# hhergeth/CudaTracerLib

Measured on AMD Instinct MI355X. Metric: Mrays/s at 1920x1080, 267 spp (steps), depth-8; achieved HBM GB/s vs peak, higher is better.
Workload: dtype f32; 1 GPU; synthetic-SM 1920x1080, 1 spp/step, depth 8, NEE on, 2000 instances x icosphere(4)/boxes, 8631000 instanced triangles; rough_transmittance=the reference's 3-D lookup on every call (bit-equal frames), framebuffer_reduce=none (1 GPU)

## Files before the change

cudatracerlib_amd/build.py:

```python
import hashlib, os, subprocess, sys, glob, tempfile

HERE = os.path.dirname(os.path.abspath(__file__))
CSRC = os.path.join(HERE, "csrc")
OUT = os.path.join(HERE, "libctl_amd.so")
SRCS = ["kernels.hip", "shade_basic.hip", "shade_full.hip", "shade_class_a.hip", "shade_class_b.hip", "shade_class_c.hip", "shade_class_p.hip", "shade_class_g.hip", "shade_class_g_wf.hip", "shade_class_p_wf.hip", "shade_class_a_wf.hip", "shade_class_b_wf.hip", "shade_class_c_wf.hip", "shade_basic_wf.hip", "shade_full_wf.hip", "megakernel.hip", "prim_tracer.hip", "traversal_probe.hip", "shading_eval_basic.hip", "shading_eval_full.hip", "shading_eval_partials.hip", "image_pipeline.hip", "nlm_filter.hip", "block_sampler.hip", "tracer.hip", "scene_update.hip", "flat_refit.hip", "capi.hip", "scene_builder.cpp", "scene_checks.cpp", "geometry_hash.cpp", "bvh_builder.cpp", "sbvh_builder.cpp", "flatten.cpp", "mitsuba_loader.cpp", "image_io.cpp", "jpeg_decode.cpp", "mesh_io.cpp", "scene_cache.cpp", "comm.cpp"]
FLAGS = ["-O3", "-std=c++17", "--offload-arch=gfx950", "-fPIC", "-ffp-contract=off", "-munsafe-fp-atomics",
         "-Wall", "-Wno-unused-function", "-Wno-unused-variable", "-pthread"]


KNOBS_OUT = os.path.join(HERE, "libctl_knobs.so")


def _flag_key(defines=()):
    return hashlib.sha256(("\0".join(sorted(defines)) + "\1" + os.environ.get("CTL_BUILD_EXTRA_FLAGS", "")).encode()).hexdigest()[:16]


def _object_dir(out):
    if out is None:
        return os.path.join(HERE, "build")
    return os.path.join(os.environ.get("TMPDIR") or tempfile.gettempdir(), "ctl_build_" + os.path.splitext(os.path.basename(out))[0])


def stale(target=None, defines=()):
    target = target or OUT
    if not os.path.exists(target):
        return True
    key = os.path.join(_object_dir(None if target == OUT else target), "flags.key")
    if not os.path.exists(key) or open(key).read().strip() != _flag_key(defines):
        return True
    t = os.path.getmtime(target)
    deps = glob.glob(os.path.join(CSRC, "*")) + [os.path.join(HERE, "..", "include", "ctl_amd.h"), __file__]
    return any(os.path.getmtime(d) > t for d in deps)


def build(force=False, verbose=True, out=None, defines=()):
    if not force and not stale(out, defines):
        return out or OUT
    hipcc = os.environ.get("HIPCC", "/opt/rocm/bin/hipcc")
    objs = []
    bdir = _object_dir(out)
    os.makedirs(bdir, exist_ok=True)
    procs = []
    for s in SRCS:
        o = os.path.join(bdir, s + ".o")
        cmd = [hipcc] + FLAGS + os.environ.get("CTL_BUILD_EXTRA_FLAGS", "").split() + ["-D" + d for d in defines] + (["-x", "hip"] if s.endswith(".cpp") else []) + ["-c", os.path.join(CSRC, s), "-o", o]
        if verbose:
            print(" ".join(cmd), flush=True)
        procs.append((s, subprocess.Popen(cmd)))
        objs.append(o)
    bad = [s for s, p in procs if p.wait() != 0]
    if bad:
        raise RuntimeError("hipcc failed for: " + ", ".join(bad))
    target = OUT if out is None else out
    cmd = [hipcc, "--offload-arch=gfx950", "-shared", "-o", target] + objs + ["-pthread", "-lz", "-ldl"]
    if verbose:
        print(" ".join(cmd), flush=True)
    subprocess.check_call(cmd)
    with open(os.path.join(bdir, "flags.key"), "w") as f:
        f.write(_flag_key(defines) + "\n")
    return target


if __name__ == "__main__":
    args = [a for a in sys.argv[1:] if a != "--force"]
    out = None; defines = []
    while args:
        a = args.pop(0)
        if a == "--out": out = os.path.abspath(args.pop(0))
        elif a.startswith("-D"): defines.append(a[2:])
    build(force="--force" in sys.argv, out=out, defines=defines, verbose=False)
    if out is None:
        build(force="--force" in sys.argv, out=KNOBS_OUT, defines=["CTL_MEASUREMENT_KNOBS"], verbose=False)
```

cudatracerlib_amd/csrc/shade_basic.hip:

```cpp
#define CTL_SHADE_NAME basic
#define CTL_SHADE_FEATURES 0
#ifndef CTL_BASIC_SHADE_BLOCK
#define CTL_BASIC_SHADE_BLOCK 256
#endif
#define CTL_SHADE_BLOCK CTL_BASIC_SHADE_BLOCK
#ifndef CTL_BASIC_SHADE_WAVES
#define CTL_BASIC_SHADE_WAVES 4
#endif
#define CTL_SHADE_WAVES CTL_BASIC_SHADE_WAVES
#ifndef CTL_BASIC_SORT_WINDOW
#define CTL_BASIC_SORT_WINDOW 256
#endif
#define CTL_SHADE_SORT_WINDOW CTL_BASIC_SORT_WINDOW
#include "shade_kernel.inc"
```

cudatracerlib_amd/csrc/shade_kernel.inc:

```
#ifndef CTL_SHADE_WAVEFRONT_RULES
#define CTL_SHADE_WAVEFRONT_RULES 0
#endif
#define CTL_SHADE_CAT_(a, b, c) a##b##c
#define CTL_SHADE_CAT(a, b, c) CTL_SHADE_CAT_(a, b, c)
#if CTL_SHADE_WAVEFRONT_RULES
#define CTL_SHADE_KERNEL CTL_SHADE_CAT(k_shade_, CTL_SHADE_NAME, _wf)
#define CTL_SHADE_LAUNCH CTL_SHADE_CAT(launch_shade_, CTL_SHADE_NAME, _wf)
#else
#define CTL_SHADE_KERNEL CTL_SHADE_CAT(k_shade_, CTL_SHADE_NAME, )
#define CTL_SHADE_LAUNCH CTL_SHADE_CAT(launch_shade_, CTL_SHADE_NAME, )
#endif
#if defined(CTL_SHADE_WAVES) && CTL_SHADE_WAVES > 0
#define CTL_SHADE_ATTR __attribute__((amdgpu_waves_per_eu(CTL_SHADE_WAVES, CTL_SHADE_WAVES)))
#else
#define CTL_SHADE_ATTR
#endif
#ifndef CTL_SHADE_LDS_TABLES
#define CTL_SHADE_LDS_TABLES 12
#endif
#ifndef CTL_SHADE_KEYS
#define CTL_SHADE_KEYS 0xFFFFu
#elif !defined(CTL_SHADE_MODELS)
#define CTL_SHADE_MODELS CTL_SHADE_KEYS
#endif
#ifdef CTL_SHADE_CLASS
#define CTL_SHADE_CLASSED 1
#define CTL_FMATH_OUTLINE
#define CTL_LIGHT_INLINE
#else
#define CTL_SHADE_CLASSED 0
#endif
#define CTL_HAS_KEY(k) ((((unsigned)(CTL_SHADE_KEYS)) >> (k)) & 1u)
#include "kernels.h"
#include "shading.h"
#include "compaction.h"

namespace ctl {

__global__ __launch_bounds__(CTL_SHADE_BLOCK) CTL_SHADE_ATTR void CTL_SHADE_KERNEL(dev_scene S, wave_queues Q, pass_params P, int depth, ctl_pixel_data* __restrict__ image) {
    __shared__ uint32_t s_cnt[3][kWideBlock / 64]; __shared__ uint32_t s_base[3];
#if CTL_SHADE_LDS_TABLES
    scene_tables_to_lds<CTL_SHADE_BLOCK>(S);
#endif
    const int cur = (depth - 1) & 1, nxt = depth & 1;
    const path_soa& A = Q.path[cur];
    const path_soa& B = Q.path[nxt];
#if CTL_SHADE_CLASSED
    const uint32_t n = Q.class_counts[depth * 8 + CTL_SHADE_CLASS];
#else
    const uint32_t n = Q.counts[(depth - 1) * 4 + 0];
#endif
    uint32_t* n_next = &Q.counts[depth * 4 + 0];
    uint32_t* n_shadow = &Q.counts[depth * 4 + 1];
    uint32_t* n_final = &Q.counts[depth * 4 + 2];
    const uint32_t* occ_prev = Q.sh_occ[(depth - 1) & 1];
    float4* sh_o = Q.sh_o[depth & 1]; float4* sh_d = Q.sh_d[depth & 1];

    const uint32_t n_round = (n + (CTL_SHADE_BLOCK - 1u)) & ~(CTL_SHADE_BLOCK - 1u);
    for (uint32_t j = blockIdx.x * CTL_SHADE_BLOCK + threadIdx.x; j < n_round; j += gridDim.x * CTL_SHADE_BLOCK) {
        bool active = j < n;
        uint32_t i = j;
#ifndef CTL_SHADE_SORT_WINDOW
#define CTL_SHADE_SORT_WINDOW CTL_SHADE_BLOCK
#endif
#if CTL_SHADE_CLASSED
        i = active ? Q.class_order[CTL_SHADE_CLASS][j] : 0u;
#else
        if (CTL_SHADE_SORT_WINDOW > 0) {
            constexpr uint32_t kWin = CTL_SHADE_SORT_WINDOW > 0 ? CTL_SHADE_SORT_WINDOW : 64, kGroups = CTL_SHADE_BLOCK / kWin;
            __shared__ uint32_t s_hist[kGroups][64]; __shared__ uint16_t s_perm[CTL_SHADE_BLOCK];
            const uint32_t grp = threadIdx.x / kWin, lane_w = threadIdx.x % kWin;
            if (threadIdx.x < kGroups * 64) s_hist[threadIdx.x >> 6][threadIdx.x & 63] = 0;
            __syncthreads();
            uint32_t key = 63u;
            if (CTL_SHADE_FEATURES == 0 && active && P.key_from_traversal) key = Q.mat_key[i];
            else if (active) {
                const int tri = __float_as_int(Q.hit[i].w);
                key = 0u;
                if (tri >= 0) {
                    const uint32_t mi = S.node_info[Q.hit_node[i]].x + tri_mat_index(S, tri);
                    key = min((S.mats[mi].bsdf_type & 15u) << 2 | (mi & 3u), 62u);
                }
            }
            const uint32_t rank = atomicAdd(&s_hist[grp][key], 1u);
            __syncthreads();
            uint32_t before = 0;
            for (uint32_t k = 0; k < key; k++) before += s_hist[grp][k];
            s_perm[grp * kWin + before + rank] = (uint16_t)lane_w;
            __syncthreads();
            const uint32_t src = s_perm[threadIdx.x];
            const uint32_t j2 = j - lane_w + src;
            active = j2 < n;
            i = j2;
        }
#endif
        bool alive = false, want_shadow = false, terminated = false;
        f3 cl(0.0f), cf(0.0f), directF(0.0f), new_o(0.0f), new_d(0.0f), last_nor(0.0f), sh_org(0.0f), sh_dir(0.0f);
        float bsdf_pdf_out = 0.0f, sh_tmax = 0.0f; uint32_t pixel = 0, d1 = 0, d2 = 0, pass_b = 0; bool specular = false; float2 px = make_float2(0.f, 0.f);
        if (active) {
            const float4 ro = A.ray_o[i], rd = A.ray_d[i], thr = A.thr[i], rad = A.rad[i], nor = A.nor[i], pend = A.pend[i];
            float4 hit = Q.hit[i]; const int hnode = Q.hit_node[i];
            if (P.u16_bary && __float_as_int(hit.w) >= 0) {
                hit.y = (float)(uint16_t)(hit.y * 65535) / 65535.0f; hit.z = (float)(uint16_t)(hit.z * 65535) / 65535.0f;
            }
            px = A.px[i];
            pixel = __float_as_uint(rad.w);
            const uint32_t packed = __float_as_uint(nor.w);
            pass_b = (packed >> 16) & 0xffu;
            const uint32_t n1 = CTL_SAMPLER_NUM_SEQUENCES * CTL_SAMPLER_SEQUENCE_LENGTH;
            sampler rng{ P.t1 + pass_b * n1, P.t2 + pass_b * n1, pixel, packed & 0xffu, (packed >> 8) & 0xffu };
            bool specularBounce = ((packed >> 24) & kFlagSpecular) != 0;
            cl = f3(rad.x, rad.y, rad.z); cf = f3(thr.x, thr.y, thr.z);
            float brdf_scattering_pdf = thr.w;
            last_nor = f3(nor.x, nor.y, nor.z);
            const uint32_t sidx = __float_as_uint(pend.w);
            if (sidx != kNoShadow && !occ_prev[sidx]) cl = cl + f3(pend.x, pend.y, pend.z);
            const f3 r_o(ro.x, ro.y, ro.z), r_d(rd.x, rd.y, rd.z);
            const int tri = __float_as_int(hit.w);
            if (depth == 1 && P.depth_buffer) {
                const uint32_t dx = pixel % P.width, dy = pixel / P.width;
                if (dx < P.depth_w && dy < P.depth_h) {
                    const float z = clampf(hit.x, P.depth_near, P.depth_far);
                    P.depth_buffer[(size_t)P.depth_w * dy + dx] = (P.depth_far / (P.depth_far - P.depth_near) * z - P.depth_far * P.depth_near / (P.depth_far - P.depth_near)) / z;
                }
            }
            if (tri >= 0 && (CTL_SHADE_KEYS & 0xFFFEu)) {
                bsdf_rec b;
                b.eta = 1.0f; b.sampled_type = 0; b.type_mask = kEAll;
                b.dg.P = r_o + hit.x * r_d;
                fill_dg(S, hit.y, hit.z, tri, hnode, b.dg);
                b.wi = b.dg.sys.to_local(-r_d);
                const uint4 ninfo = S.node_info[hnode];
#ifdef CTL_SHADE_PROBE_MAT_L1
                const ctl_material& mat = S.mats[min((uint32_t)hnode + CTL_SHADE_PROBE_MAT_L1 - 1u, S.n_materials_probe - 1u)];
#else
                const ctl_material& mat = S.mats[ninfo.x + tri_mat_index(S, tri)];
#endif
#if CTL_SHADE_FEATURES & 32
                if (mat.map_kind != CTL_MAP_NONE) sample_normal_map(mat, b.dg);
#endif
                if (mat.two_sided && b.wi.z < 0) { b.dg.n = -b.dg.n; b.dg.sys.n = -b.dg.sys.n; b.wi.z *= -1.0f; }
                const uint32_t nli = mat.node_light_index;
                if (nli != 0xffffffffu) {
                    const uint32_t li = nli == 0 ? ninfo.y : ninfo.z;
                    const ctl_light& light = scene_lights(S)[li];
                    float misWeight = 1.0f;
                    if (!(!P.direct || depth == 1 || specularBounce)) {
                        const float direct_pdf = light_pdf_direct(light, r_d, last_nor, b.dg.n, hit.x) * pdf_emitter(S, li);
                        misWeight = power_heuristic(brdf_scattering_pdf, direct_pdf);
                    }
#if CTL_SHADE_WAVEFRONT_RULES
                    cl = cl + misWeight * light_eval(S, light, b.dg.P, b.dg.sys.n, -r_d) * cf;
#else
                    cl = cl + misWeight * cf * light_eval(S, light, b.dg.P, b.dg.sys.n, -r_d);
#endif
                }
#if CTL_SHADE_WAVEFRONT_RULES
                bool surviveRR = true;
                if (depth - 1 >= P.rr_start_depth) {
                    const float q = max3c(cf);
                    if (rng.next1() < q) cf = sdiv(cf, q); else surviveRR = false;
                }
                if (depth != P.max_path_length && surviveRR) {
                    const f3 f = bsdf_sample_top(mat, b, brdf_scattering_pdf, rng.next2());
                    new_o = b.dg.P; new_d = b.dg.sys.to_world(b.wo);
                    specularBounce = (b.sampled_type & kEDelta) != 0;
                    if (P.direct && (mat.combined_type & kESmooth) && S.num_lights) {
                        f2 sl = rng.next2();
                        float lpdf; const int li = sample_emitter_reuse(S, lpdf, sl.x);
                        if (li >= 0) {
                            direct_rec dr; dr.ref = b.dg.P; dr.refN = b.dg.sys.n;
                            f3 value = light_sample_direct(S, scene_lights(S)[li], dr, sl);
                            if (dr.pdf != 0) { dr.pdf *= lpdf; value = sdiv(value, lpdf); } else value = f3(0.0f);
                            if (!is_zero(value)) {
                                b.type_mask = kEAll & ~kEDelta; b.wo = b.dg.sys.to_local(dr.d);
                                const f3 bsdfVal = bsdf_f_top(mat, b);
                                const float bp = bsdf_pdf_top(mat, b);
                                const float directPdf = dr.measure == kMeasureArea ? dr.pdf * dr.dist / fabsf(dot(dr.n, dr.d)) : dr.pdf;
                                directF = cf * value * bsdfVal * power_heuristic(directPdf, bp);
                                want_shadow = true;
                                sh_org = dr.ref; sh_dir = dr.d; sh_tmax = dr.dist * (1 - S.eps);
                            }
                        }
                    }
                    last_nor = uchar2_to_normal(normal_to_uchar2(b.dg.sys.n));
                    cf = cf * f;
                    alive = !is_zero(cf);
                }
#else
                const f3 f = bsdf_sample_top(mat, b, brdf_scattering_pdf, rng.next2());
                last_nor = b.dg.sys.n;
                new_o = b.dg.P; new_d = b.dg.sys.to_world(b.wo);
                specularBounce = (b.sampled_type & kEDelta) != 0;
                if (P.direct && (mat.combined_type & kESmooth)) {
                    if (S.num_lights) {
                        const f2 sl = rng.next2();
                        float lpdf; const int li = sample_emitter(S, lpdf, sl.x);
                        if (li >= 0) {
                            direct_rec dr; dr.ref = b.dg.P; dr.refN = b.dg.sys.n;
                            const f3 value = light_sample_direct(S, scene_lights(S)[li], dr, rng.next2());
                            if (!is_zero(value)) {
                                b.wo = b.dg.sys.to_local(dr.d); b.type_mask = kEAll & ~kEDelta;
                                const f3 bsdfVal = bsdf_f_top(mat, b);
                                if (!is_zero(bsdfVal)) {
                                    float weight = 1.0f;
                                    if (dr.measure != kMeasureDiscrete) {
                                        const float bp = bsdf_pdf_top(mat, b);
                                        const float directPdf = (dr.measure == kMeasureArea ? dr.pdf * dr.dist / fabsf(dot(dr.n, dr.d)) : dr.pdf) * lpdf;
                                        weight = power_heuristic(directPdf, bp);
                                    }
                                    directF = cf * sdiv(value * bsdfVal * weight, lpdf);
                                    want_shadow = true;
                                    sh_org = dr.ref; sh_dir = dr.d; sh_tmax = dr.dist - S.eps;
                                }
                            }
                        }
                    }
                }
                if (P.direct && (mat.combined_type & kESmooth)) cl = cl + cf * f3(0.0f);
                cf = cf * f;
                alive = true;
                if (is_zero(cf)) alive = false;
                if (alive && depth >= P.max_path_length) alive = false;
                if (alive && depth > P.rr_start_depth && !specularBounce) {
                    const float q = max3c(cf);
                    if (rng.next1() >= q) alive = false; else cf = sdiv(cf, q);
                }
#endif
            }
#if CTL_SHADE_FEATURES & 8
            else if (CTL_HAS_KEY(0) && S.env_map_index != 0xffffffffu) {
                const ctl_light& light = scene_lights(S)[S.env_map_index];
                float misWeight = 1.0f;
                if (!(!P.direct || depth == 1 || specularBounce)) {
                    const float direct_pdf = env_pdf_direct(S, light, r_d) * pdf_emitter(S, S.env_map_index);
                    misWeight = power_heuristic(brdf_scattering_pdf, direct_pdf);
                }
                cl = cl + misWeight * cf * env_eval(S, light, r_d);
            }
#endif
            else if (CTL_HAS_KEY(0) && tri < 0) cl = cl + cf * f3(0.0f);
            terminated = !alive;
            specular = specularBounce; bsdf_pdf_out = brdf_scattering_pdf; d1 = rng.d1; d2 = rng.d2;
        }
        const block_slots bs = block_append3(n_shadow, want_shadow, n_next, alive, n_final, terminated && want_shadow, s_cnt, s_base);
        const uint32_t sslot = bs.s[0], nslot = bs.s[1], fslot = bs.s[2];
        if (!active) continue;
        if (want_shadow) { sh_o[sslot] = make_float4(sh_org.x, sh_org.y, sh_org.z, S.eps); sh_d[sslot] = make_float4(sh_dir.x, sh_dir.y, sh_dir.z, sh_tmax); }
        if (alive) {
            B.ray_o[nslot] = make_float4(new_o.x, new_o.y, new_o.z, S.eps);
            B.ray_d[nslot] = make_float4(new_d.x, new_d.y, new_d.z, 3.402823466e+38f);
            B.thr[nslot] = make_float4(cf.x, cf.y, cf.z, bsdf_pdf_out);
            B.rad[nslot] = make_float4(cl.x, cl.y, cl.z, __uint_as_float(pixel));
            B.nor[nslot] = make_float4(last_nor.x, last_nor.y, last_nor.z, __uint_as_float((d1 % CTL_SAMPLER_SEQUENCE_LENGTH) | ((d2 % CTL_SAMPLER_SEQUENCE_LENGTH) << 8) | (pass_b << 16)    | ((specular ? kFlagSpecular : 0u) << 24)));
            B.pend[nslot] = make_float4(directF.x, directF.y, directF.z, __uint_as_float(want_shadow ? sslot : kNoShadow));
            B.px[nslot] = px;
        } else if (want_shadow) {
            Q.fin.rad[fslot] = make_float4(cl.x, cl.y, cl.z, __uint_as_float(sslot));
            Q.fin.dir[fslot] = make_float4(directF.x, directF.y, directF.z, 0.0f);
            Q.fin.px[fslot] = make_float4(px.x, px.y, __uint_as_float(pixel), __uint_as_float(pass_b));
        } else {
            add_sample_ordered(P, image, pixel, pass_b, px.x, px.y, cl);
        }
    }
}

void CTL_SHADE_LAUNCH(const launch_ctx& lc, const dev_scene& S, const wave_queues& Q, const pass_params& P, int depth, ctl_pixel_data* image) {
#ifndef CTL_SHADE_GRID_WAVES
#define CTL_SHADE_GRID_WAVES 4
#endif
    hipLaunchKernelGGL(CTL_SHADE_KERNEL, dim3(lc.grid_blocks / 8 * (kWideBlock / CTL_SHADE_BLOCK) * CTL_SHADE_GRID_WAVES / 4), dim3(CTL_SHADE_BLOCK), 0, lc.stream, S, Q, P, depth, image);
}

}
```

Before: 3250 Mrays/s.

## Park long-lived shade values in LDS to raise basic shade occupancy

Adds an LDS parking area in the basic shade kernel. Long-lived per-path values (cl, cf, new_d, px, pass) are stored to shared memory and reloaded around the BSDF and light sampling code, which lowers VGPR pressure. The waves-per-EU target goes from 4 to 5, and SLP vectorization is disabled for all device code. This trades extra LDS traffic and some LDS capacity for higher occupancy. The global flag also changes codegen for every other kernel.

```diff
diff --git a/cudatracerlib_amd/build.py b/cudatracerlib_amd/build.py
--- a/cudatracerlib_amd/build.py
+++ b/cudatracerlib_amd/build.py
@@ -5,7 +5,8 @@
 OUT = os.path.join(HERE, "libctl_amd.so")
 SRCS = ["kernels.hip", "shade_basic.hip", "shade_full.hip", "shade_class_a.hip", "shade_class_b.hip", "shade_class_c.hip", "shade_class_p.hip", "shade_class_g.hip", "shade_class_g_wf.hip", "shade_class_p_wf.hip", "shade_class_a_wf.hip", "shade_class_b_wf.hip", "shade_class_c_wf.hip", "shade_basic_wf.hip", "shade_full_wf.hip", "megakernel.hip", "prim_tracer.hip", "traversal_probe.hip", "shading_eval_basic.hip", "shading_eval_full.hip", "shading_eval_partials.hip", "image_pipeline.hip", "nlm_filter.hip", "block_sampler.hip", "tracer.hip", "scene_update.hip", "flat_refit.hip", "capi.hip", "scene_builder.cpp", "scene_checks.cpp", "geometry_hash.cpp", "bvh_builder.cpp", "sbvh_builder.cpp", "flatten.cpp", "mitsuba_loader.cpp", "image_io.cpp", "jpeg_decode.cpp", "mesh_io.cpp", "scene_cache.cpp", "comm.cpp"]
 FLAGS = ["-O3", "-std=c++17", "--offload-arch=gfx950", "-fPIC", "-ffp-contract=off", "-munsafe-fp-atomics",
-         "-Wall", "-Wno-unused-function", "-Wno-unused-variable", "-pthread"]
+         "-Wall", "-Wno-unused-function", "-Wno-unused-variable", "-pthread",
+         "-Xarch_device", "-fno-slp-vectorize"]
 
 
 KNOBS_OUT = os.path.join(HERE, "libctl_knobs.so")
diff --git a/cudatracerlib_amd/csrc/shade_basic.hip b/cudatracerlib_amd/csrc/shade_basic.hip
--- a/cudatracerlib_amd/csrc/shade_basic.hip
+++ b/cudatracerlib_amd/csrc/shade_basic.hip
@@ -5,11 +5,16 @@
 #endif
 #define CTL_SHADE_BLOCK CTL_BASIC_SHADE_BLOCK
 #ifndef CTL_BASIC_SHADE_WAVES
-#define CTL_BASIC_SHADE_WAVES 4
+#define CTL_BASIC_SHADE_WAVES 5
 #endif
 #define CTL_SHADE_WAVES CTL_BASIC_SHADE_WAVES
 #ifndef CTL_BASIC_SORT_WINDOW
 #define CTL_BASIC_SORT_WINDOW 256
 #endif
 #define CTL_SHADE_SORT_WINDOW CTL_BASIC_SORT_WINDOW
+#ifndef CTL_BASIC_SHADE_PARK
+#define CTL_BASIC_SHADE_PARK 1
+#endif
+#define CTL_SHADE_PARK CTL_BASIC_SHADE_PARK
+#define CTL_SHADE_GRID_WAVES CTL_BASIC_SHADE_WAVES
 #include "shade_kernel.inc"
diff --git a/cudatracerlib_amd/csrc/shade_kernel.inc b/cudatracerlib_amd/csrc/shade_kernel.inc
--- a/cudatracerlib_amd/csrc/shade_kernel.inc
+++ b/cudatracerlib_amd/csrc/shade_kernel.inc
@@ -31,14 +31,32 @@
 #define CTL_SHADE_CLASSED 0
 #endif
 #define CTL_HAS_KEY(k) ((((unsigned)(CTL_SHADE_KEYS)) >> (k)) & 1u)
+#ifndef CTL_SHADE_PARK
+#define CTL_SHADE_PARK 0
+#endif
+#if CTL_SHADE_PARK && CTL_SHADE_WAVEFRONT_RULES
+#error "CTL_SHADE_PARK is written for the default path rules"
+#endif
 #include "kernels.h"
 #include "shading.h"
 #include "compaction.h"
 
 namespace ctl {
 
+#if CTL_SHADE_PARK
+__device__ __forceinline__ uint32_t park_lane() { uint32_t t = threadIdx.x; asm volatile("" : "+v"(t)); return t; }
+#define CTL_PARK3(k, v) (s_park[k][threadIdx.x] = (v).x, s_park[(k) + 1][threadIdx.x] = (v).y, s_park[(k) + 2][threadIdx.x] = (v).z)
+#define CTL_UNPARK3(k, v) ((v) = f3(s_park[k][park_lane()], s_park[(k) + 1][park_lane()], s_park[(k) + 2][park_lane()]))
+#else
+#define CTL_PARK3(k, v) ((void)0)
+#define CTL_UNPARK3(k, v) ((void)0)
+#endif
+enum { kParkCl = 0, kParkCf = 3, kParkNewD = 6, kParkPx = 9, kParkPass = 11, kParkWords = 12 };
 __global__ __launch_bounds__(CTL_SHADE_BLOCK) CTL_SHADE_ATTR void CTL_SHADE_KERNEL(dev_scene S, wave_queues Q, pass_params P, int depth, ctl_pixel_data* __restrict__ image) {
     __shared__ uint32_t s_cnt[3][kWideBlock / 64]; __shared__ uint32_t s_base[3];
+#if CTL_SHADE_PARK
+    __shared__ float s_park[kParkWords][CTL_SHADE_BLOCK];
+#endif
 #if CTL_SHADE_LDS_TABLES
     scene_tables_to_lds<CTL_SHADE_BLOCK>(S);
 #endif
@@ -107,6 +125,9 @@
             pixel = __float_as_uint(rad.w);
             const uint32_t packed = __float_as_uint(nor.w);
             pass_b = (packed >> 16) & 0xffu;
+#if CTL_SHADE_PARK
+            s_park[kParkPx][threadIdx.x] = px.x; s_park[kParkPx + 1][threadIdx.x] = px.y; s_park[kParkPass][threadIdx.x] = __uint_as_float(pass_b);
+#endif
             const uint32_t n1 = CTL_SAMPLER_NUM_SEQUENCES * CTL_SAMPLER_SEQUENCE_LENGTH;
             sampler rng{ P.t1 + pass_b * n1, P.t2 + pass_b * n1, pixel, packed & 0xffu, (packed >> 8) & 0xffu };
             bool specularBounce = ((packed >> 24) & kFlagSpecular) != 0;
@@ -115,6 +136,7 @@
             last_nor = f3(nor.x, nor.y, nor.z);
             const uint32_t sidx = __float_as_uint(pend.w);
             if (sidx != kNoShadow && !occ_prev[sidx]) cl = cl + f3(pend.x, pend.y, pend.z);
+            CTL_PARK3(kParkCl, cl); CTL_PARK3(kParkCf, cf);
             const f3 r_o(ro.x, ro.y, ro.z), r_d(rd.x, rd.y, rd.z);
             const int tri = __float_as_int(hit.w);
             if (depth == 1 && P.depth_buffer) {
@@ -152,7 +174,9 @@
 #if CTL_SHADE_WAVEFRONT_RULES
                     cl = cl + misWeight * light_eval(S, light, b.dg.P, b.dg.sys.n, -r_d) * cf;
 #else
+                    CTL_UNPARK3(kParkCl, cl); CTL_UNPARK3(kParkCf, cf);
                     cl = cl + misWeight * cf * light_eval(S, light, b.dg.P, b.dg.sys.n, -r_d);
+                    CTL_PARK3(kParkCl, cl);
 #endif
                 }
 #if CTL_SHADE_WAVEFRONT_RULES
@@ -192,6 +216,7 @@
                 last_nor = b.dg.sys.n;
                 new_o = b.dg.P; new_d = b.dg.sys.to_world(b.wo);
                 specularBounce = (b.sampled_type & kEDelta) != 0;
+                CTL_PARK3(kParkNewD, new_d);
                 if (P.direct && (mat.combined_type & kESmooth)) {
                     if (S.num_lights) {
                         const f2 sl = rng.next2();
@@ -209,6 +234,7 @@
                                         const float directPdf = (dr.measure == kMeasureArea ? dr.pdf * dr.dist / fabsf(dot(dr.n, dr.d)) : dr.pdf) * lpdf;
                                         weight = power_heuristic(directPdf, bp);
                                     }
+                                    CTL_UNPARK3(kParkCf, cf);
                                     directF = cf * sdiv(value * bsdfVal * weight, lpdf);
                                     want_shadow = true;
                                     sh_org = dr.ref; sh_dir = dr.d; sh_tmax = dr.dist - S.eps;
@@ -217,7 +243,8 @@
                         }
                     }
                 }
-                if (P.direct && (mat.combined_type & kESmooth)) cl = cl + cf * f3(0.0f);
+                CTL_UNPARK3(kParkCf, cf);
+                if (P.direct && (mat.combined_type & kESmooth)) { CTL_UNPARK3(kParkCl, cl); cl = cl + cf * f3(0.0f); CTL_PARK3(kParkCl, cl); }
                 cf = cf * f;
                 alive = true;
                 if (is_zero(cf)) alive = false;
@@ -236,18 +263,24 @@
                     const float direct_pdf = env_pdf_direct(S, light, r_d) * pdf_emitter(S, S.env_map_index);
                     misWeight = power_heuristic(brdf_scattering_pdf, direct_pdf);
                 }
+                CTL_UNPARK3(kParkCl, cl); CTL_UNPARK3(kParkCf, cf);
                 cl = cl + misWeight * cf * env_eval(S, light, r_d);
-            }
-#endif
-            else if (CTL_HAS_KEY(0) && tri < 0) cl = cl + cf * f3(0.0f);
+                CTL_PARK3(kParkCl, cl);
+            }
+#endif
+            else if (CTL_HAS_KEY(0) && tri < 0) { CTL_UNPARK3(kParkCl, cl); CTL_UNPARK3(kParkCf, cf); cl = cl + cf * f3(0.0f); CTL_PARK3(kParkCl, cl); }
             terminated = !alive;
             specular = specularBounce; bsdf_pdf_out = brdf_scattering_pdf; d1 = rng.d1; d2 = rng.d2;
         }
         const block_slots bs = block_append3(n_shadow, want_shadow, n_next, alive, n_final, terminated && want_shadow, s_cnt, s_base);
         const uint32_t sslot = bs.s[0], nslot = bs.s[1], fslot = bs.s[2];
         if (!active) continue;
+#if CTL_SHADE_PARK
+        CTL_UNPARK3(kParkCl, cl); px = make_float2(s_park[kParkPx][park_lane()], s_park[kParkPx + 1][park_lane()]); pass_b = __float_as_uint(s_park[kParkPass][park_lane()]);
+#endif
         if (want_shadow) { sh_o[sslot] = make_float4(sh_org.x, sh_org.y, sh_org.z, S.eps); sh_d[sslot] = make_float4(sh_dir.x, sh_dir.y, sh_dir.z, sh_tmax); }
         if (alive) {
+            CTL_UNPARK3(kParkNewD, new_d);
             B.ray_o[nslot] = make_float4(new_o.x, new_o.y, new_o.z, S.eps);
             B.ray_d[nslot] = make_float4(new_d.x, new_d.y, new_d.z, 3.402823466e+38f);
             B.thr[nslot] = make_float4(cf.x, cf.y, cf.z, bsdf_pdf_out);
```

Result: faster. 3361 Mrays/s (median of 6 runs) (+3.4%).
